# vice87/gam-ngs

Hardware: AMD Instinct MI355X
Metric: GCUPS (higher is better)
Workload: dtype int32 (fast blocks: exact packed-f16 offsets from per-lane int32 bases, two tasks per register; results bit-identical to the reference's int64 DP)

## Files before the change

### gam_ngs_amd/csrc/gamdp_dev.h

```cpp
#pragma once
#include <stdint.h>

namespace gamdp {

typedef uint32_t u32;
typedef uint64_t u64;

constexpr int SEQ_PAD_BASES = 4096;

#ifndef GAMDP_WAVES_PER_SIMD
#define GAMDP_WAVES_PER_SIMD 5
#endif

struct DevTask {
    const u32* a2;
    const u32* an;
    const u32* b2;
    const u32* bn;
    int64_t a_base;
    int64_t b_base;
    int64_t end_a;
    int32_t alen, blen;
    int32_t begin_a, begin_b;
    int32_t X;
    int32_t band;
    u32 flags;
    u32 res_idx;
    u64 ops_off;
    u64 ops_cap;
};

enum : u32 { TF_FORCE_START = 1, TF_FORCE_END = 2, TF_WANT_OPS = 4,
             TF_DIAG_SKIP_TRACEBACK = 8 ,
             TF_NO_DIRFREE = 16 ,
             TF_DIAG_COUNT_MAT = 32 ,
             TF_PADDING = 64 ,
             TF_CALL_N = 128  };

#ifdef GAMDP_DIAG
constexpr u32 TF_LIVE_MASK = ~0u;
#else
constexpr u32 TF_LIVE_MASK = ~(u32)(TF_DIAG_SKIP_TRACEBACK | TF_NO_DIRFREE | TF_DIAG_COUNT_MAT);
#endif

struct DevResult {
    int32_t begin_a, begin_b;
    int32_t score;
    u32 n_match, length;
    int32_t first_a, first_b, last_a, last_b;
    u32 flags;
};

struct LaunchParams {
    const DevTask* tasks;
    u32 n_tasks;
    u32* cursor;
    DevResult* results;
    uint8_t* ops_buf;
    u32* scratch;
    u64 slot_words;
    u64 dir_words;
    u32 ypad;
    u64 ckpt_off;
    u64 bnd_off;
    u32 flags;
    u32 prio_R, prio_from;
    u32* stats;
};
enum : int { LS_UNITS = 0, LS_DIRFREE, LS_PACKED_TOP, LS_PACKED_TOP_MIXED, LS_STRIPS, LS_TOP_WANTED, LS_SKIP_TESTS, LS_SKIP_TESTED, LS_SKIP_GROUPS, LS_SKIP_SHORT, LS_COUNT = 12 };
constexpr u32 LP_WALK_SKIP_DIAG = 32;
constexpr u32 LP_WALK_SIDE_BY_SIDE = 1;
constexpr u32 LP_NO_PACKED_TOP = 2;
constexpr u32 LP_NO_PACKED_TOP_MIXED = 16;
constexpr u32 LP_WALK_PRIO_SHIFT = 8;

enum KernelId : int {
    K_C17_CE4 = 0,
    K_C17_CE4_N,
    K_C5_CE0,
    K_C5_CE0_N,
    K_P17_CE4,
    K_O19_CE15,
    K_Q19_CE15,
    K_Q19_CE15_N,
    K_GEN_C2, K_GEN_C3, K_GEN_C5, K_GEN_C9, K_GEN_C17,
    K_WIDE,
    K_COUNT
};

constexpr int FAMILY_COLS[5] = {2, 3, 5, 9, 17};
constexpr int band_cols(const u32 band)
{
    for (int k = 0; k < 4; k++) if (2 * (u64)band + 1 <= 64u * (u64)FAMILY_COLS[k]) return FAMILY_COLS[k];
    return 17;
}
constexpr int cols_index(const int cols)
{
    for (int k = 0; k < 4; k++) if (FAMILY_COLS[k] == cols) return k;
    return 4;
}
static_assert(K_GEN_C3 == K_GEN_C2 + 1 && K_GEN_C5 == K_GEN_C2 + 2 && K_GEN_C9 == K_GEN_C2 + 3 && K_GEN_C17 == K_GEN_C2 + 4,
              "K_GEN_C2 .. K_GEN_C17: contiguous, in the order of FAMILY_COLS");
constexpr int gen_kernel_id(const int cols) { return (int)K_GEN_C2 + cols_index(cols); }

#if defined(__HIPCC__)
#define GAMDP_HD __host__ __device__
#else
#define GAMDP_HD
#endif

constexpr u32 PAT_OFF = 0x2000u, PAT_MIN = 0x0400u, PAT_MAX = 0x7BFFu - 21u;
GAMDP_HD inline u32 pat_encode(int rel) { return (PAT_OFF + (u32)rel) & 0xFFFFu; }
GAMDP_HD inline int pat_decode(u32 p16) { return (int)(int16_t)(uint16_t)p16 - (int)PAT_OFF; }

GAMDP_HD inline int preflight_hd(u64 alen, u64 blen, u64 band, u64 begin_a, u64 end_a, u64 begin_b, u64 end_b, bool fs, bool fe,
                                 u64* X_out, u64* cells_out)
{
    constexpr int64_t MAXGAP = 10;
    enum { S_OK = 0, S_EMPTY = 1, S_OOR = 2, S_INVALID = 3 };
    auto mn = [](int64_t x, int64_t y) { return x < y ? x : y; };
    *X_out = 0;
    *cells_out = 0;
    if (end_b < begin_b) return S_EMPTY;
    if (begin_a >= (1ull << 31) - 65536) return S_INVALID;
    const int64_t lo = ((int64_t)begin_a - (int64_t)band) > 0 ? ((int64_t)begin_a - (int64_t)band) : 0, hi = (int64_t)begin_a + (int64_t)band;
    if (begin_b >= blen) {
        bool any;
        if (!fs) any = lo < (int64_t)alen;
        else any = (lo <= mn(hi, MAXGAP)) || lo < (int64_t)alen;
        return any ? S_OOR : S_INVALID;
    }
    if (end_b >= blen) end_b = blen - 1;
    u64 X = end_b - begin_b + 1;
    const u64 lim = alen + band - begin_a;
    if (lim < X) X = lim;
    if (X > 500000) X = 500000;
    if (X == 0) return S_INVALID;
    const u64 Y = 2 * band + 1;
    *X_out = X;
    *cells_out = X * Y;
    if (fs) {
        const int64_t up = mn(hi, MAXGAP);
        if (lo <= up && up >= (int64_t)alen) return S_OOR;
    }
    if (begin_a > alen + band) {
        bool found = false;
        if (!fe) found = begin_a + (X - 1) - band <= end_a;
        {
            const bool ge = end_a >= begin_a + band;
            const int64_t i0 = ge ? (int64_t)(end_a - (begin_a + band)) : 0;
            const int64_t j0 = ge ? (int64_t)(2 * band) : (int64_t)(2 * band) - (int64_t)(begin_a + band - end_a);
            if (j0 >= 0 && (u64)i0 < X) {
                const int64_t kmax = mn((int64_t)X - 1 - i0, j0);
                if (!fe) found = true;
                else if (X >= (u64)MAXGAP + 1 && (u64)(i0 + kmax) >= X - 1 - (u64)MAXGAP) found = true;
            }
        }
        return found ? S_OOR : S_EMPTY;
    }
    return S_OK;
}

GAMDP_HD inline bool npre_window_has_n(const u32* pre, int64_t len, bool rc, u64 off, int64_t lo, int64_t hi)
{
    if (pre == nullptr) return false;
    const int64_t o_lo = (int64_t)off + (lo > 0 ? lo : 0), o_hi = ((int64_t)off + hi < len - 1) ? (int64_t)off + hi : len - 1;
    if (o_lo > o_hi) return false;
    const int64_t f_lo = rc ? len - 1 - o_hi : o_lo, f_hi = rc ? len - 1 - o_lo : o_hi;
    return pre[(f_hi / 256) + 1] != pre[f_lo / 256];
}
GAMDP_HD inline bool call_touches_n(const u32* pre_a, int64_t alen, bool a_rc, u64 a_off, const u32* pre_b, int64_t blen, bool b_rc, u64 b_off,
                                    int64_t band, int64_t begin_a, int64_t begin_b, int64_t X, int64_t margin)
{
    return npre_window_has_n(pre_a, alen, a_rc, a_off, begin_a - band - margin, begin_a + X - 1 + band + margin) ||
           npre_window_has_n(pre_b, blen, b_rc, b_off, begin_b - margin, begin_b + X - 1 + margin);
}

struct DevBlk { int32_t m_begin, m_end, s_begin, s_end; };
struct DevMB {
    const u32 *a2, *an;
    const u32 *b2, *bn;
    const u32 *b2rc, *bnrc;
    u64 mlen, slen;
    u64 m_start, s_start, s_end;
    u64 align_thr;
    u32 first_blk, n_blocks;
    u32 audit_first;
    u32 rows;
    u32 try_rev;
    u32 has_n;
    const u32 *npre_a, *npre_b;
    u32 max_x;
    u64 slot_off[2];
    u64 slot_words, dir_words;
    u64 ckpt_off, bnd_off;
};
struct ChainOut { u32 n_dp; u32 state; u32 t_begin, t_end; u32 hw, hw_twin; u32 t_end_att[2]; u32 t_begin2; u32 pad; };
struct ChainWin { u64 begin_a, end_a, begin_b, end_b; u32 X; u32 info; };
struct ChainSync { u32 verdict[2]; u32 n[2]; u32 fin; u32 cancel; u32 t_begin; u32 hw[2]; u32 t_end[2]; u32 t_begin2; };
struct ChainParams {
    const DevMB* mbs; const DevBlk* blks; u32 n_mbs;
    u32 n_twins;
    ChainSync* sync;
    u32 first_mb;
    u32* cursor;
    DevResult* audit; ChainOut* out;
    ChainWin* win;
    u32* scratch; u32 ypad; u32 band;
    u32 max_rows;
    DevResult* host_audit; ChainOut* host_out; u32* host_done; u32 epoch;
    ChainWin* host_win;
    u32 skew_call;
    int32_t n_margin;
    u32 n_by_contig;
};
int chain_slots_per_workgroup();

struct KernelInfo {
    KernelId id;
    const char* name;
    int cols;
    u32 band;
    int tasks_per_wave;
    int waves_per_cu;
    bool n_aware;
    bool dirfree;
    bool two_dir_images;
    int dir_block_words;
    int ckpt_words;
    int bnd_words;
    void (*kernel)(LaunchParams);
};
extern const KernelInfo kernel_info[K_COUNT];

inline u64 dir_words_for(const KernelInfo& ki, const u64 X, const u64 band)
{
    const u64 Y = 2 * band + 1;
    if (ki.id == K_WIDE) return X * Y;
    const u64 C = (u64)ki.cols, LE = (Y - 1) / C;
    const u64 extra = ki.tasks_per_wave > 1 ? 3 : 0;
    return ((X - 1 + LE) / 16 + 1 + extra) * (u64)ki.dir_block_words;
}
struct SlotGeom { u64 dir_words; u32 ypad; u64 slot_words, ckpt_off, bnd_off; };
inline SlotGeom slot_geom(const KernelInfo& ki, const u64 max_dir_words, const u32 max_band)
{
    SlotGeom g;
    g.ypad = ((2 * max_band + 2 + 63) / 64) * 64;
    g.dir_words = ((max_dir_words + 63) / 64) * 64;
    const u64 tpw = (u64)ki.tasks_per_wave;
    u64 ckpt_words = 0, bnd_words = 0;
    if (tpw > 1 || ki.dirfree) {
        const u64 nblk = g.dir_words / (u64)ki.dir_block_words + 1;
        ckpt_words = (nblk / 4 + 2) * (u64)ki.ckpt_words;
        bnd_words = (nblk + 4) * (u64)ki.bnd_words;
    }
    const u64 sides_end = (ki.two_dir_images ? 2 * g.dir_words : g.dir_words) + 4ull * g.ypad * tpw;
    g.slot_words = sides_end + ckpt_words + bnd_words;
    g.ckpt_off = ckpt_words ? sides_end : 0;
    g.bnd_off = g.ckpt_off + ckpt_words;
    return g;
}

struct KernelFamily {
    const void* kernel[5];
    const char* name[5];
    unsigned threads;
};
const KernelFamily& score_family();
const KernelFamily& carry_family();
const KernelFamily& chain_carry_family();
const KernelFamily& chain_gen_family();

enum ChainNBit : int {
    CHAIN_N_UNREPORTED,
    CHAIN_N_BY_WINDOW,
    CHAIN_N_EVERY_DP
};
struct ChainKernel {
    const char* name;
    const void* kernel;
    int cols;
    unsigned threads;
    const KernelInfo* slots;
    bool twins;
    ChainNBit n_bit;
};
const ChainKernel& chain2_kernel(bool has_n);
inline ChainKernel family_chain_kernel(const KernelFamily& f, const int cols, const KernelInfo* slots, const bool twins, const ChainNBit n_bit)
{
    return ChainKernel{f.name[cols_index(cols)], f.kernel[cols_index(cols)], cols, f.threads, slots, twins, n_bit};
}

int launch_align(int kid, const LaunchParams& p, unsigned n_slots, unsigned dyn_lds, void* stream);
int launch_wide(const LaunchParams& p, unsigned n_slots, void* stream);
constexpr int WIDE_WORKGROUPS_PER_CU = 8;

struct alignas(16) ScoreRec {
    int32_t score, end_a, end_b;
    u32 info;
};
struct ScoreParams {
    const DevTask* tasks;
    u32 n_tasks;
    u32* cursor;
    ScoreRec* results;
};

struct CarryParams {
    const DevTask* tasks;
    u32 n_tasks;
    u32* cursor;
    DevResult* results;
};
constexpr u32 CARRY_COLS_SHIFT = 16;


}
```

### gam_ngs_amd/csrc/kernel_pair.inc

```
#ifndef GAMDP_PACKED_TOP
#define GAMDP_PACKED_TOP 1
#endif
typedef _Float16 h2 __attribute__((ext_vector_type(2)));
__device__ __forceinline__ h2 as_h2(u32 x) { return __builtin_bit_cast(h2, x); }
__device__ __forceinline__ u32 as_u(h2 x) { return __builtin_bit_cast(u32, x); }
constexpr u32 PK_NINF = 0xFC00FC00u;
constexpr u32 PK_PINF = 0x7C007C00u;

__device__ __forceinline__ u32 pk(const _Float16 lo, const _Float16 hi) { const h2 v = {lo, hi}; return as_u(v); }
__device__ __forceinline__ _Float16 lo_of(const u32 v) { return as_h2(v).x; }
__device__ __forceinline__ _Float16 hi_of(const u32 v) { return as_h2(v).y; }

__device__ __forceinline__ _Float16 g4_to_h(const int g4, const int base)
{
    if (g4 <= NEG / 2) return lo_of(PK_NINF);
    return (_Float16)(float)((g4 >> 2) - base);
}
__device__ __forceinline__ int h_to_g4(const _Float16 h, const int base)
{
    const float f = (float)h;
    if (!(f > -60000.0f)) return NEG;
    if (!(f < 60000.0f)) return 0;
    return 4 * ((int)f + base);
}

typedef unsigned short us2 __attribute__((ext_vector_type(2)));
constexpr u32 PAT_OFF2 = PAT_OFF * 0x00010001u;
__device__ __forceinline__ u32 pat_add(const u32 a, const u32 b) { return __builtin_bit_cast(u32, __builtin_bit_cast(us2, a) + __builtin_bit_cast(us2, b)); }
__device__ __forceinline__ u32 pat_sub(const u32 a, const u32 b) { return __builtin_bit_cast(u32, __builtin_bit_cast(us2, a) - __builtin_bit_cast(us2, b)); }
__device__ __forceinline__ u32 pk16(const int lo, const int hi) { return ((u32)lo & 0xFFFFu) | ((u32)hi << 16); }
__device__ __forceinline__ u32 pat_lo(const u32 v) { return v & 0xFFFFu; }
__device__ __forceinline__ u32 pat_hi(const u32 v) { return v >> 16; }
__device__ __forceinline__ u32 g4_to_pat(const int g4, const int base)
{
    if (g4 <= NEG / 2) return 0xFC00u;
    return pat_encode((g4 >> 2) - base);
}
__device__ __forceinline__ int pat_to_g4(const u32 p, const int base)
{
    if (p & 0x8000u) return NEG;
    return 4 * (pat_decode(p) + base);
}
__device__ __forceinline__ u32 h2_to_pat(const u32 v)
{
    const h2 lim = {(_Float16)16000.0f, (_Float16)16000.0f};
    const h2 c = __builtin_elementwise_min(__builtin_elementwise_max(as_h2(v), -lim), lim);
    return pat_add(pk16((int)(short)c.x, (int)(short)c.y), PAT_OFF2);
}

template <int C, int LPT>
struct PairFmt {
    typedef Strip<LPT, true> ST;
    static constexpr bool GRP = (LPT == QL);
    static constexpr u32 CK_LANE = GRP ? 24u : (u32)LANE_WORDS<C>;
    static_assert(!GRP || C + 4 <= 24, "checkpoint row of the eight-task kernel");
    static constexpr u32 CK_ROWS = 64u * CK_LANE;
    static constexpr u32 CK_WORDS = GRP ? CK_ROWS : CK_ROWS + 128;
    static constexpr u32 BND_VALS = ST::BND_WORDS;
    static constexpr u32 BND_WORDS = GRP ? ST::BND_WORDS : ST::BND_WORDS + 2u * ST::NB;
    static constexpr int RC = 4;
};
__shared__ u32 s_ringB2[RING_B + ROWS];
__shared__ u32 s_pcap[QT][2][20];

__device__ __forceinline__ u32 pk_sel(const u32 codeA, const u32 codeB) { return 0x000C000Cu | (codeA << 8) | ((4u + codeB) << 24); }
__device__ __forceinline__ u32 pk_tab(const u32 codeb) { return 0x44444444u + (0x03u << (codeb * 8u)); }
__device__ __forceinline__ u32 pat_sel(const u32 codeA, const u32 codeB) { return 0x0C000C00u | codeA | ((4u + codeB) << 16); }
__device__ __forceinline__ u32 pat_tab(const u32 codeb) { return 0x0C0C0C0Cu + (0x09u << (codeb * 8u)); }

__device__ __forceinline__ u32 code2_at(gcptr p2, int64_t idx) { return (p2[idx >> 4] >> ((idx & 15) * 2)) & 3u; }

__shared__ u32 s_oB2[QT][64 + ROWS];
template <int C, int LPT, bool PAT = false>
struct PRing {
    static_assert(!PAT || LPT == 64, "the pattern format is the two-task kernel's");
    static __device__ __forceinline__ u32 sel(const u32 codeA, const u32 codeB) { return PAT ? pat_sel(codeA, codeB) : pk_sel(codeA, codeB); }
    static __device__ __forceinline__ u32 tab(const u32 codeb) { return PAT ? pat_tab(codeb) : pk_tab(codeb); }
    typedef typename std::conditional<LPT == 64, const u32*, const uint16_t*>::type APtr;
    static constexpr int SZ = QRing<C>::SZ;
    static __device__ __forceinline__ void put_a(const int sub, const int k, const u32 codeA, const u32 codeB)
    {
        if constexpr (LPT == 64) RingA<C>::put(k, sel(codeA, codeB));
        else {
            const u32 pos = (u32)k % (u32)SZ;
            const uint16_t v = (uint16_t)(codeA | ((4u + codeB) << 8));
            s_oA16[sub][pos] = v;
            if (pos < ROWS) s_oA16[sub][pos + SZ] = v;
        }
    }
    static __device__ __forceinline__ void put_b(const int sub, const int k, const u32 ta, const u32 tb)
    {
        if constexpr (LPT == 64) {
            const int pb = k & (RING_B - 1);
            s_ringB[pb] = ta; s_ringB2[pb] = tb;
            if (pb < ROWS) { s_ringB[pb + RING_B] = ta; s_ringB2[pb + RING_B] = tb; }
        } else {
            const int pb = k & 63;
            s_qB[sub][pb] = ta; s_oB2[sub][pb] = tb;
            if (pb < ROWS) { s_qB[sub][pb + 64] = ta; s_oB2[sub][pb + 64] = tb; }
        }
    }
    static __device__ __forceinline__ APtr a_lane(const int tau0, const int lane)
    {
        if constexpr (LPT == 64) return s_ringA + (u32)((tau0 + (C - 1) * (lane + 1)) >> 4) % (u32)RingA<C>::COLS;
        else return s_oA16[lane >> 4] + (u32)(tau0 + (C - 1) * ((lane & (QL - 1)) + 1)) % (u32)SZ;
    }
    static __device__ __forceinline__ u32 a_read(APtr p, const int r)
    {
        if constexpr (LPT == 64) return p[r * RingA<C>::COLS];
        else return __builtin_amdgcn_perm(0x0C0C0C0Cu, (u32)p[r], 0x01040004u);
    }
    static __device__ __forceinline__ const u32* b_lane(const int tau0, const int lane, const int half)
    {
        if constexpr (LPT == 64) return (half ? s_ringB2 : s_ringB) + ((tau0 - lane) & (RING_B - 1));
        else return (half ? s_oB2[lane >> 4] : s_qB[lane >> 4]) + ((tau0 - (lane & (QL - 1))) & 63);
    }
    template <int C2>
    static __device__ __forceinline__ _Float16 cap_pick(const int wlane, const int half, const u32 (&Lp)[C2], const int idx)
    {
        const int lane = wlane & (LPT - 1);
        if constexpr (LPT == 64) {
            u32* const cb = (u32*)s_cap[half][lane & 1];
#pragma unroll
            for (int c = 0; c < C2; ++c) cb[c] = Lp[c];
            const u32 v = cb[idx];
            return half ? hi_of(v) : lo_of(v);
        } else {
            u32* const cb = s_pcap[wlane >> 4][lane & 1];
#pragma unroll
            for (int c = 0; c < C2; ++c) cb[c] = Lp[c];
            return __builtin_bit_cast(_Float16, reinterpret_cast<const uint16_t*>(cb)[2 * idx + half]);
        }
    }
    template <int C2>
    static __device__ __forceinline__ u32 cap_pick_pat(const int wlane, const int half, const u32 (&Lp)[C2], const int idx)
    {
        static_assert(LPT == 64, "the pattern format is the two-task kernel's");
        u32* const cb = (u32*)s_cap[half][wlane & 1];
#pragma unroll
        for (int c = 0; c < C2; ++c) cb[c] = Lp[c];
        const u32 v = cb[idx];
        return half ? pat_hi(v) : pat_lo(v);
    }
    static constexpr u32 MARK_A = 13u, MARK_B = 9u;
    template <bool MARK = false>
    static __device__ __forceinline__ void produce(const int T, const int lane, const u32 awA, const u32 awB, const u32 bwA, const u32 bwB, const int km1A = 0, const int km1B = 0)
    {
        const int r = lane & (QL - 1);
        if (LPT == QL || lane < ROWS) {
            const int k = T + (C - 1) * LPT + r;
            u32 cA = (awA >> (2 * r)) & 3u, cB = (awB >> (2 * r)) & 3u;
            if constexpr (MARK) { cA = (k == km1A) ? MARK_A : cA; cB = (k == km1B) ? MARK_B : cB; }
            put_a(lane >> 4, k, cA, cB);
            put_b(lane >> 4, T + r, tab((bwA >> (2 * r)) & 3u), tab((bwB >> (2 * r)) & 3u));
        }
    }
    template <bool MARK = false>
    static __device__ __forceinline__ void prime(const Tk& ta, const Tk& tb, const int blk, const int lane, const int km1A = 0, const int km1B = 0)
    {
        const int T0 = blk * ROWS, tl = lane & (LPT - 1), sub = lane >> 4;
        const int64_t A0a = ta.a_base + ta.begin_a - ta.band, A0b = tb.a_base + tb.begin_a - tb.band;
        for (int k = T0 + tl; k < T0 + ROWS + (C - 1) * LPT; k += LPT) {
            u32 cA = code2_at(ta.a2, A0a + k), cB = code2_at(tb.a2, A0b + k);
            if constexpr (MARK) { cA = (k == km1A) ? MARK_A : cA; cB = (k == km1B) ? MARK_B : cB; }
            put_a(sub, k, cA, cB);
        }
        const int64_t Ba = ta.b_base + ta.begin_b, Bb = tb.b_base + tb.begin_b;
        for (int k = T0 - (LPT - 1) + tl; k <= T0 + ROWS - 1; k += LPT) put_b(sub, k, tab(code2_at(ta.b2, Ba + k)), tab(code2_at(tb.b2, Bb + k)));
    }
};

template <int C, bool HASN, bool UNTAGGED, int LPT>
__device__ __forceinline__ void single_prime(const Tk& t, const int blk, const int wlane, u32 (&W)[C + 15])
{
    typedef Ring<C, LPT, HASN> RG;
    const int T0 = blk * ROWS, lane = wlane & (LPT - 1), sub = wlane >> 4;
    const int64_t A0 = t.a_base + t.begin_a - t.band, BB = t.b_base + t.begin_b;
    for (int k = T0 + lane; k < T0 + ROWS + (C - 1) * LPT; k += LPT) RG::put_a(sub, k, code2_at(t.a2, A0 + k), false);
    for (int k = T0 - (LPT - 1) + lane; k <= T0 + ROWS - 1; k += LPT)
        RG::put_b(sub, k, enc_b<HASN>(code2_at(t.b2, BB + k), false) - (UNTAGGED ? RING_TAG<HASN> : 0u));
    const int64_t s0 = A0 + (int64_t)(C - 1) * lane + T0;
    const u32 ab = fetch16(t.a2, s0), ab2 = (C - 1 > 16) ? fetch16(t.a2, s0 + 16) : 0u;
#pragma unroll
    for (int k = 0; k < C - 1; ++k) W[k] = (k < 16) ? enc_a<HASN>((ab >> (2 * k)) & 3u, false) : enc_a<HASN>((ab2 >> (2 * (k - 16))) & 3u, false);
#pragma unroll
    for (int k = C - 1; k < C + 15; ++k) W[k] = 0;
}

template <int C, int LPT>
__device__ __forceinline__ void ck_store(gptr ck, const int wlane, const u32 (&Lp)[C], const int baseA, const int baseB)
{
    typedef PairFmt<C, LPT> FMT;
    if constexpr (FMT::GRP) {
        const u32 rA = (u32)lane_shl1<LPT>(baseA, baseA), rB = (u32)lane_shl1<LPT>(baseB, baseB);
        gptr row = ck + (u32)wlane * FMT::CK_LANE;
#pragma unroll
        for (int g = 0; g < 6; ++g) {
            auto w = [&](const int i) -> u32 { return i < C ? Lp[i < C ? i : 0] : (i == C ? (u32)baseA : (i == C + 1 ? (u32)baseB : (i == C + 2 ? rA : (i == C + 3 ? rB : 0u)))); };
            const u32x4 q = {w(4 * g), w(4 * g + 1), w(4 * g + 2), w(4 * g + 3)};
            *(g4ptr)(row + 4 * g) = q;
        }
    } else {
        img_store<C, true>(ck, wlane, Lp);
        ck[FMT::CK_ROWS + wlane] = (u32)baseA;
        ck[FMT::CK_ROWS + 64 + wlane] = (u32)baseB;
    }
}

template <int C, int LPT>
__device__ __forceinline__ int cap_limit(const Tk& t, const int lane) { return max(0, min(C, t.Y - C * lane)); }
template <int LPT>
__device__ __forceinline__ void cap_table(const int wlane, const int half, const int E0, const int R0, const int P0, const int L0)
{
    if ((wlane & (LPT - 1)) == 0) {
        const int4 e = {E0, R0, P0, L0};
        *reinterpret_cast<int4*>(s_captab[LPT == 64 ? 0 : wlane >> 4][half]) = e;
    }
}
template <int C, int CE, int LPT, bool LAST, bool PAT = false>
__device__ __forceinline__ void side_capture(const int wlane, const int half, const int T, const int base, const u32 (&Lp)[C], const int cap_max, giptr const cap_slot)
{
    const int lane = wlane & (LPT - 1);
    const int4 e = *reinterpret_cast<const int4*>(s_captab[LPT == 64 ? 0 : wlane >> 4][half]);
    const int cE = e.x - (C - 1) * lane - T;
    if ((u32)cE < (u32)cap_max && T <= e.y + lane) {
        if constexpr (PAT) {
            const u32 vE = PRing<C, LPT>::cap_pick_pat(wlane, half, Lp, cE);
            cap_slot[e.z - lane + T] = pat_decode(vE) + base + 8 * (lane - e.x - T);
        } else {
            const _Float16 vE = PRing<C, LPT>::cap_pick(wlane, half, Lp, cE);
            cap_slot[e.z - lane + T] = (int)(float)vE + base + 8 * (lane - e.x - T);
        }
    }
    if constexpr (LAST) {
        if (T == e.y + lane && cap_max > 0) {
            giptr const lp = cap_slot + (e.w + C * lane);
            const int k1 = base - 16 * e.y - 8 * C * lane;
            auto put = [&](const int c) __attribute__((always_inline)) {
                if constexpr (PAT) lp[c] = pat_decode(half ? pat_hi(Lp[c]) : pat_lo(Lp[c])) + (k1 - 8 * c);
                else lp[c] = (int)(float)(half ? hi_of(Lp[c]) : lo_of(Lp[c])) + (k1 - 8 * c);
            };
#pragma unroll
            for (int c = 0; c <= CE; ++c) put(c);
            if (cap_max == C) {
#pragma unroll
                for (int c = CE + 1; c < C; ++c) put(c);
            }
        }
    }
}

template <int C, int CE, bool END, int LPT = 64>
__device__ __noinline__ void pair_range(BlockState<C>* sta, BlockState<C>* stb, const Tk* tpa, const Tk* tpb, const int blk_begin_, const int blk_end_, const int wlane)
{
    static_assert(CE >= 0 && CE < C - 1 && (LPT == QL || (C - 1) % 16 == 0), "band 512 on 64 lanes (transposed ring A) or band 150 on 16");
    constexpr bool PAT = (LPT == 64);
    typedef PRing<C, LPT, PAT> PR;
    const Tk ta = load_tk<LPT>(tpa), tb = load_tk<LPT>(tpb);
    const int blk_begin = uni(blk_begin_), blk_end = uni(blk_end_);
    const int lane = wlane & (LPT - 1);
    const int LE = (ta.Y - 1) / C;
    u32 Lp[C], W[C + 15];
    int baseA, baseB;
    u32 Lin, dL, dR;
    {
        baseA = (sta->Lp[0] <= NEG / 2) ? 0 : (sta->Lp[0] >> 2);
        baseB = (stb->Lp[0] <= NEG / 2) ? 0 : (stb->Lp[0] >> 2);
        const int lA = __shfl_up(baseA, 1, LPT), lB = __shfl_up(baseB, 1, LPT), rA = __shfl_down(baseA, 1, LPT), rB = __shfl_down(baseB, 1, LPT);
        const bool hasL = lane >= 1 && lane <= LE, hasR = lane < LE;
        if constexpr (PAT) {
#pragma unroll
            for (int c = 0; c < C; ++c) Lp[c] = g4_to_pat(sta->Lp[c], baseA) | (g4_to_pat(stb->Lp[c], baseB) << 16);
            Lin = g4_to_pat(sta->Lin, baseA) | (g4_to_pat(stb->Lin, baseB) << 16);
            dL = hasL ? pk16(lA - baseA, lB - baseB) : 0u;
            dR = hasR ? pk16(rA - baseA, rB - baseB) : 0u;
        } else {
#pragma unroll
            for (int c = 0; c < C; ++c) Lp[c] = pk(g4_to_h(sta->Lp[c], baseA), g4_to_h(stb->Lp[c], baseB));
            Lin = pk(g4_to_h(sta->Lin, baseA), g4_to_h(stb->Lin, baseB));
            dL = hasL ? pk((_Float16)(float)(lA - baseA), (_Float16)(float)(lB - baseB)) : 0u;
            dR = hasR ? pk((_Float16)(float)(rA - baseA), (_Float16)(float)(rB - baseB)) : 0u;
        }
        const int T0 = blk_begin * ROWS;
        const int64_t sa = ta.a_base + ta.begin_a - ta.band + (int64_t)(C - 1) * lane + T0, sb = tb.a_base + tb.begin_a - tb.band + (int64_t)(C - 1) * lane + T0;
        const u32 wa = fetch16(ta.a2, sa), wb = fetch16(tb.a2, sb);
        const u32 wa2 = (C - 1 > 16) ? fetch16(ta.a2, sa + 16) : 0u, wb2 = (C - 1 > 16) ? fetch16(tb.a2, sb + 16) : 0u;
#pragma unroll
        for (int k = 0; k < C - 1; ++k)
            W[k] = (k < 16) ? PR::sel((wa >> (2 * k)) & 3u, (wb >> (2 * k)) & 3u) : PR::sel((wa2 >> (2 * (k - 16))) & 3u, (wb2 >> (2 * (k - 16))) & 3u);
#pragma unroll
        for (int k = C - 1; k < C + 15; ++k) W[k] = 0;
    }
    PR::prime(ta, tb, blk_begin, wlane);

    const int64_t iAa = ta.a_base + ta.begin_a - ta.band + (C - 1) * LPT, iBa = ta.b_base + ta.begin_b;
    const int64_t iAb = tb.a_base + tb.begin_a - tb.band + (C - 1) * LPT, iBb = tb.b_base + tb.begin_b;
    gcptr paA = ta.a2 + (iAa >> 4), pbA = ta.b2 + (iBa >> 4), paB = tb.a2 + (iAb >> 4), pbB = tb.b2 + (iBb >> 4);
    const u32 shaA = (u32)(iAa & 15) * 2u, shbA = (u32)(iBa & 15) * 2u, shaB = (u32)(iAb & 15) * 2u, shbB = (u32)(iBb & 15) * 2u;
    u32 aA_lo = paA[blk_begin + 1], aA_hi = paA[blk_begin + 2], bA_lo = pbA[blk_begin + 1], bA_hi = pbA[blk_begin + 2];
    u32 aB_lo = paB[blk_begin + 1], aB_hi = paB[blk_begin + 2], bB_lo = pbB[blk_begin + 1], bB_hi = pbB[blk_begin + 2];
    asm volatile("" : "+v"(aA_lo), "+v"(aA_hi), "+v"(bA_lo), "+v"(bA_hi), "+v"(aB_lo), "+v"(aB_hi), "+v"(bB_lo), "+v"(bB_hi));
    [[maybe_unused]] const h2 three = {(_Float16)3.0f, (_Float16)3.0f};
    const bool no_up = lane == LE;
    typedef Strip<LPT, true> ST;
    typedef PairFmt<C, LPT> FMT;
    constexpr int SPAN = (C - 1) * 21 + FMT::RC * ROWS * 21;
    static_assert(!PAT || ((int)PAT_OFF - (SPAN + 21) >= (int)PAT_MIN && (int)PAT_OFF + SPAN + 21 <= (int)PAT_MAX), "the live patterns of a group stay normal, finite f16 numbers");
    constexpr int NB = ST::NB, FI = ST::FI;
    const int sshift = uni(ta.sshift);
    const bool edge = ST::opens_strip(wlane, sshift);
    const u32 my_slot = ST::slot_of(wlane, sshift);
    const u64 edge_mask = __ballot(edge);
    u32* const s_bnd = ST::staging();
    u32* const sb = s_bnd + my_slot;
    gptr const ckpt = ta.ckpt, bnd = ta.bnd;
    int xkeep = (int)PK_NINF;
    const int prio_R = uni(ta.prio_R), prio_nblk = uni(ta.prio_nblk);
    const int cap_max = END ? cap_limit<C, LPT>(ta, lane) : 0;
    giptr const cap_slot = (giptr)unip(ta.dir);
    if constexpr (END) {
        cap_table<LPT>(wlane, 0, ta.eaRel, ta.X - 1, (int)(ta.adh - cap_slot) - ta.iA, (int)(ta.lastrow - cap_slot));
        cap_table<LPT>(wlane, 1, tb.eaRel, tb.X - 1, (int)(tb.adh - cap_slot) - tb.iA, (int)(tb.lastrow - cap_slot));
    }
    constexpr bool ROT = (C + 15 == 32);
    auto block_body = [&](auto phase, const int blk) __attribute__((always_inline)) {
        constexpr int WO = ROT ? 16 * decltype(phase)::value : 0;
#define WX(i) (ROT ? (((i) + WO) & 31) : (i))
        const int T = (blk + 1) * ROWS, tau0 = blk * ROWS;
        if (prio_R != 0 && (blk & 7) == 0) set_prio_by_remaining(prio_nblk - blk, prio_R);
        const u32 aA_nx = paA[blk + 3], bA_nx = pbA[blk + 3], aB_nx = paB[blk + 3], bB_nx = pbB[blk + 3];
        PR::produce(T, wlane, __builtin_amdgcn_alignbit(aA_hi, aA_lo, shaA), __builtin_amdgcn_alignbit(aB_hi, aB_lo, shaB),
                    __builtin_amdgcn_alignbit(bA_hi, bA_lo, shbA), __builtin_amdgcn_alignbit(bB_hi, bB_lo, shbB));
        if ((blk & 3) == 0) ck_store<C, LPT>(ckpt + (u64)(blk >> 2) * FMT::CK_WORDS, wlane, Lp, baseA, baseB);
        if constexpr (!FMT::GRP) {
            if (edge) {
                gptr bb = bnd + (u64)blk * FMT::BND_WORDS + FMT::BND_VALS;
                bb[my_slot] = (u32)baseA;
                bb[NB + my_slot] = (u32)baseB;
            }
        }
        const typename PR::APtr ringA_lane = PR::a_lane(tau0, wlane);
        const u32* const rbA = PR::b_lane(tau0, wlane, 0);
        const u32* const rbB = PR::b_lane(tau0, wlane, 1);
        {
            u32 tA[2], tB[2];
            u32 m[3], D[2];
            u32 L = Lin, x = PK_NINF, Lrecv = Lin;
            W[WX(C - 1)] = PR::a_read(ringA_lane, 0);
            tA[0] = rbA[0]; tB[0] = rbB[0];
            W[WX(C)] = PR::a_read(ringA_lane, 1);
            tA[1] = rbA[1]; tB[1] = rbB[1];
            auto do_perm = [&](const int g) __attribute__((always_inline)) {
                const int r = g / C, c = g % C;
                m[g % 3] = __builtin_amdgcn_perm(tB[r & 1], tA[r & 1], W[WX(r + c)]);
            };
            auto do_fma = [&](const int g) __attribute__((always_inline)) {
                if constexpr (PAT) D[g % 2] = m[g % 3] + Lp[g % C];
                else D[g % 2] = as_u(__builtin_elementwise_fma(as_h2(m[g % 3]), three, as_h2(Lp[g % C])));
            };
            auto do_max = [&](const int g) __attribute__((always_inline)) {
                const int c = g % C;
                h2 U = as_h2((c < C - 1) ? Lp[(c < C - 1) ? c + 1 : c] : x);
                if (c == CE) U = as_h2(no_up ? PK_NINF : as_u(U));
                L = as_u(__builtin_elementwise_maximum(__builtin_elementwise_maximum(as_h2(D[g % 2]), U), as_h2(L)));
                Lp[c] = L;
            };
            do_perm(0); do_perm(1); do_fma(0);
            __builtin_amdgcn_sched_barrier(0);
            static_for<ROWS>([&](auto rc) __attribute__((always_inline)) {
                constexpr int r = decltype(rc)::value;
#pragma unroll
                for (int c = 0; c < C; ++c) {
                    const int g = r * C + c;
                    if (c == 0) {
                        L = Lin; Lrecv = Lin;
                        do_fma(g + 1);
                        do_max(g);
                        do_perm(g + 2);
                    } else {
                        do_max(g);
                        if (g + 1 < ROWS * C) do_fma(g + 1);
                        if (g + 2 < ROWS * C) do_perm(g + 2);
                    }
                    if (c == 2) xkeep = lane_shl1<LPT>(xkeep, (int)Lp[0]);
                    if (c == 3) {
                        x = PAT ? pat_add((u32)xkeep, dR) : as_u(as_h2((u32)xkeep) + as_h2(dR));
                        lds_store2_masked<4 * (r % FI) * NB, 4 * (NB * FI + (r % FI) * NB)>(sb, Lrecv, Lp[0], edge_mask);
                    }
                    __builtin_amdgcn_sched_barrier(0);
                }
                if constexpr (r + 2 < ROWS) { W[WX(C + 1 + r)] = PR::a_read(ringA_lane, r + 2); tA[r & 1] = rbA[r + 2]; tB[r & 1] = rbB[r + 2]; }
                Lin = (u32)lane_shr1<LPT>((int)Lin, (int)L);
                Lin = PAT ? pat_add(Lin, dL) : as_u(as_h2(Lin) + as_h2(dL));
                __builtin_amdgcn_sched_barrier(0);
                if constexpr (END) {
                    side_capture<C, CE, LPT, true, PAT>(wlane, 0, tau0 + r, baseA, Lp, cap_max, cap_slot);
                    side_capture<C, CE, LPT, true, PAT>(wlane, 1, tau0 + r, baseB, Lp, cap_max, cap_slot);
                }
                if ((r % FI) == FI - 1) {
                    constexpr u32 PER = 2u * NB * FI / 64u;
                    const u32 w0 = (u32)wlane * PER;
                    const u32* src = s_bnd + ST::staging_index(w0);
                    gptr bp = bnd + (u64)blk * FMT::BND_WORDS + (u32)(r / FI) * (u32)(2 * NB * FI) + w0;
#pragma unroll
                    for (u32 k = 0; k < PER; k += 4) {
                        const u32x4 v = {src[k * NB], src[(k + 1) * NB], src[(k + 2) * NB], src[(k + 3) * NB]};
                        *(g4ptr)(bp + k) = v;
                    }
                }
            });
        }
#ifdef GAMDP_DIAG
        {
            if constexpr (PAT) {
                auto mn = [](const u32 a, const u32 b) { return __builtin_bit_cast(u32, __builtin_elementwise_min(__builtin_bit_cast(us2, a), __builtin_bit_cast(us2, b))); };
                auto mx = [](const u32 a, const u32 b) { return __builtin_bit_cast(u32, __builtin_elementwise_max(__builtin_bit_cast(us2, a), __builtin_bit_cast(us2, b))); };
                u32 nIn = 0xFFFFFFFFu, xIn = 0, nOut = 0xFFFFFFFFu, xOut = 0;
#pragma unroll
                for (int c = 0; c < C; ++c) {
                    if (c <= CE) { nIn = mn(nIn, Lp[c]); xIn = mx(xIn, Lp[c]); }
                    else { nOut = mn(nOut, Lp[c]); xOut = mx(xOut, Lp[c]); }
                }
                if (lane >= 1) { nIn = mn(nIn, Lin); xIn = mx(xIn, Lin); }
                const u32 xv = pat_add((u32)xkeep, dR);
                if (blk > blk_begin) { nOut = mn(nOut, xv); xOut = mx(xOut, xv); }
                if (lane < LE) { nIn = mn(nIn, nOut); xIn = mx(xIn, xOut); }
                if (lane <= LE) {
                    if (pat_lo(nIn) < PAT_MIN || pat_lo(xIn) > PAT_MAX) ta.pos0[-1] = 1;
                    if (pat_hi(nIn) < PAT_MIN || pat_hi(xIn) > PAT_MAX) tb.pos0[-1] = 1;
                }
            } else {
            u32 mIn = 0, mOut = 0;
#pragma unroll
            for (int c = 0; c < C; ++c) {
                const u32 a = Lp[c] & 0x7FFF7FFFu;
                if (c <= CE) mIn = as_u(__builtin_elementwise_max(as_h2(mIn), as_h2(a)));
                else mOut = as_u(__builtin_elementwise_max(as_h2(mOut), as_h2(a)));
            }
            if (lane >= 1) mIn = as_u(__builtin_elementwise_max(as_h2(mIn), as_h2(Lin & 0x7FFF7FFFu)));
            const u32 xv = as_u(as_h2((u32)xkeep) + as_h2(dR)) & 0x7FFF7FFFu;
            if (blk > blk_begin) mOut = as_u(__builtin_elementwise_max(as_h2(mOut), as_h2(xv)));
            if (lane < LE) mIn = as_u(__builtin_elementwise_max(as_h2(mIn), as_h2(mOut)));
            if (lane <= LE) {
                if (!((float)lo_of(mIn) < 2040.0f)) ta.pos0[-1] = 1;
                if (!((float)hi_of(mIn) < 2040.0f)) tb.pos0[-1] = 1;
            }
            }
        }
#endif
        if constexpr (PAT) {
            if ((blk & (FMT::RC - 1)) == FMT::RC - 1 || blk + 1 == blk_end) {
                const u32 d = (lane <= LE) ? pat_sub(Lp[0], PAT_OFF2) : 0u;
                baseA += (int)(short)pat_lo(d);
                baseB += (int)d >> 16;
#pragma unroll
                for (int c = 0; c < C; ++c) Lp[c] = pat_sub(Lp[c], d);
                if (lane != 0) Lin = pat_sub(Lin, d);
                const u32 dl = (u32)lane_shr1<LPT>((int)d, (int)d);
                const u32 dr = (u32)lane_shl1<LPT>((int)d, (int)d);
                if (lane >= 1 && lane <= LE) dL = pat_sub(pat_add(dL, dl), d);
                if (lane < LE) dR = pat_sub(pat_add(dR, dr), d);
            }
        } else
        if ((blk & (FMT::RC - 1)) == FMT::RC - 1 || blk + 1 == blk_end) {
            const float fa = (float)lo_of(Lp[0]), fb = (float)hi_of(Lp[0]);
            const bool oka = fa > -60000.0f && fa < 60000.0f, okb = fb > -60000.0f && fb < 60000.0f;
            const u32 d = pk(oka ? lo_of(Lp[0]) : (_Float16)0.0f, okb ? hi_of(Lp[0]) : (_Float16)0.0f);
            baseA += oka ? (int)fa : 0;
            baseB += okb ? (int)fb : 0;
#pragma unroll
            for (int c = 0; c < C; ++c) Lp[c] = as_u(as_h2(Lp[c]) - as_h2(d));
            Lin = as_u(as_h2(Lin) - as_h2(d));
            const u32 dl = (u32)lane_shr1<LPT>((int)d, (int)d);
            const u32 dr = (u32)lane_shl1<LPT>((int)d, (int)d);
            if (lane >= 1 && lane <= LE) dL = as_u(as_h2(dL) + as_h2(dl) - as_h2(d));
            if (lane < LE) dR = as_u(as_h2(dR) + as_h2(dr) - as_h2(d));
        }
        if constexpr (!ROT) {
#pragma unroll
            for (int k = 0; k < C - 1; ++k) W[k] = W[k + ROWS];
        }
        aA_lo = aA_hi; aA_hi = aA_nx; bA_lo = bA_hi; bA_hi = bA_nx;
        aB_lo = aB_hi; aB_hi = aB_nx; bB_lo = bB_hi; bB_hi = bB_nx;
#undef WX
    };
    if constexpr (ROT) {
        int blk = blk_begin;
        for (; blk + 1 < blk_end; blk += 2) {
            block_body(std::integral_constant<int, 0>{}, blk);
            block_body(std::integral_constant<int, 1>{}, blk + 1);
        }
        if (blk < blk_end) block_body(std::integral_constant<int, 0>{}, blk);
    } else {
        for (int blk = blk_begin; blk < blk_end; ++blk) block_body(std::integral_constant<int, 0>{}, blk);
    }
    const bool dead_lane = PAT && lane > LE;
    auto back = [&](const u32 v, const int half, const int base) -> int {
        if constexpr (PAT) return dead_lane ? NEG : pat_to_g4(half ? pat_hi(v) : pat_lo(v), base);
        else return h_to_g4(half ? hi_of(v) : lo_of(v), base);
    };
#pragma unroll
    for (int c = 0; c < C; ++c) {
        sta->Lp[c] = back(Lp[c], 0, baseA); stb->Lp[c] = back(Lp[c], 1, baseB);
        sta->acc[c] = 0; stb->acc[c] = 0;
    }
    sta->Lin = back(Lin, 0, baseA); stb->Lin = back(Lin, 1, baseB);
    sta->Lout = sta->Lp[C - 1]; stb->Lout = stb->Lp[C - 1];
}

template <int C, int CE, int LPT = 64, bool FS = false>
__device__ __noinline__ void pair_top_range(BlockState<C>* sta, BlockState<C>* stb, const Tk* tpa, const Tk* tpb, const int blk_begin_, const int blk_end_, const int wlane)
{
    static_assert(CE >= 0 && CE < C - 1 && (LPT == QL || (C - 1) % 16 == 0), "band 512 on 64 lanes (transposed ring A) or band 150 on 16");
    typedef PRing<C, LPT> PR;
    const Tk ta = load_tk<LPT>(tpa), tb = load_tk<LPT>(tpb);
    const int blk_begin = uni(blk_begin_), blk_end = uni(blk_end_);
    const int lane = wlane & (LPT - 1);
    const int LE = (ta.Y - 1) / C;
    const int T0 = blk_begin * ROWS;
    const int km1A = ta.band - ta.begin_a - 1, km1B = tb.band - tb.begin_a - 1;
    const int zk = 8 * km1A, zkB = 8 * km1B;
    u32 Lp[C], W[C + 15];
    int baseA, baseB;
    u32 Lin, dL, dR;
    {
        const int rp = T0 - lane - 1, p0 = ta.begin_a + rp + C * lane - ta.band;
        const int p0B = tb.begin_a + rp + C * lane - tb.band;
        const bool dead0 = p0 < -1 && lane <= LE;
        const bool dead0B = p0B < -1 && lane <= LE;
        baseA = (sta->Lp[0] <= NEG / 2) ? 0 : (sta->Lp[0] >> 2);
        baseB = (stb->Lp[0] <= NEG / 2) ? 0 : (stb->Lp[0] >> 2);
        if (dead0) baseA = 16 * rp + 8 * C * lane;
        if (dead0B) baseB = 16 * rp + 8 * C * lane;
#pragma unroll
        for (int c = 0; c < C; ++c) {
            const bool dead = p0 + c < -1 && lane <= LE, deadB = p0B + c < -1 && lane <= LE;
            Lp[c] = pk(dead ? lo_of(PK_NINF) : g4_to_h(sta->Lp[c], baseA), deadB ? lo_of(PK_NINF) : g4_to_h(stb->Lp[c], baseB));
        }
        Lin = pk(dead0 ? lo_of(PK_NINF) : g4_to_h(sta->Lin, baseA), dead0B ? lo_of(PK_NINF) : g4_to_h(stb->Lin, baseB));
        const int lA = __shfl_up(baseA, 1, LPT), lB = __shfl_up(baseB, 1, LPT), rA = __shfl_down(baseA, 1, LPT), rB = __shfl_down(baseB, 1, LPT);
        const bool hasL = lane >= 1 && lane <= LE, hasR = lane < LE;
        dL = hasL ? pk((_Float16)(float)(lA - baseA), (_Float16)(float)(lB - baseB)) : 0u;
        dR = hasR ? pk((_Float16)(float)(rA - baseA), (_Float16)(float)(rB - baseB)) : 0u;
        const int64_t sa = ta.a_base + ta.begin_a - ta.band + (int64_t)(C - 1) * lane + T0, sb = tb.a_base + tb.begin_a - tb.band + (int64_t)(C - 1) * lane + T0;
        const u32 wa = fetch16(ta.a2, sa), wb = fetch16(tb.a2, sb);
        const u32 wa2 = (C - 1 > 16) ? fetch16(ta.a2, sa + 16) : 0u, wb2 = (C - 1 > 16) ? fetch16(tb.a2, sb + 16) : 0u;
        const int w0k = (C - 1) * lane + T0;
#pragma unroll
        for (int k = 0; k < C - 1; ++k) {
            const u32 cA = (k < 16) ? (wa >> (2 * k)) & 3u : (wa2 >> (2 * (k - 16))) & 3u, cB = (k < 16) ? (wb >> (2 * k)) & 3u : (wb2 >> (2 * (k - 16))) & 3u;
            W[k] = pk_sel((w0k + k == km1A) ? PR::MARK_A : cA, (w0k + k == km1B) ? PR::MARK_B : cB);
        }
#pragma unroll
        for (int k = C - 1; k < C + 15; ++k) W[k] = 0;
    }
    PR::template prime<true>(ta, tb, blk_begin, wlane, km1A, km1B);
    const int64_t iAa = ta.a_base + ta.begin_a - ta.band + (C - 1) * LPT, iBa = ta.b_base + ta.begin_b;
    const int64_t iAb = tb.a_base + tb.begin_a - tb.band + (C - 1) * LPT, iBb = tb.b_base + tb.begin_b;
    gcptr paA = ta.a2 + (iAa >> 4), pbA = ta.b2 + (iBa >> 4), paB = tb.a2 + (iAb >> 4), pbB = tb.b2 + (iBb >> 4);
    const u32 shaA = (u32)(iAa & 15) * 2u, shbA = (u32)(iBa & 15) * 2u, shaB = (u32)(iAb & 15) * 2u, shbB = (u32)(iBb & 15) * 2u;
    u32 aA_lo = paA[blk_begin + 1], aA_hi = paA[blk_begin + 2], bA_lo = pbA[blk_begin + 1], bA_hi = pbA[blk_begin + 2];
    u32 aB_lo = paB[blk_begin + 1], aB_hi = paB[blk_begin + 2], bB_lo = pbB[blk_begin + 1], bB_hi = pbB[blk_begin + 2];
    const h2 three = {(_Float16)3.0f, (_Float16)3.0f};
    const bool no_up = lane == LE;
    typedef Strip<LPT, true> ST;
    typedef PairFmt<C, LPT> FMT;
    constexpr int NB = ST::NB, FI = ST::FI;
    const int sshift = uni(ta.sshift);
    const bool edge = ST::opens_strip(wlane, sshift);
    const u32 my_slot = ST::slot_of(wlane, sshift);
    const u64 edge_mask = __ballot(edge);
    u32* const s_bnd = ST::staging();
    u32* const sb = s_bnd + my_slot;
    gptr const ckpt = ta.ckpt, bnd = ta.bnd;
    int xkeep = (int)PK_NINF;
    auto hf = [](const int v) -> _Float16 { return (_Float16)(float)v; };
    int g0A = baseA, g0B = baseB;
    const int cap_max = cap_limit<C, LPT>(ta, lane);
    giptr const cap_slot = (giptr)unip(ta.dir);
    cap_table<LPT>(wlane, 0, ta.band - ta.begin_a, ta.X - 1, (int)(ta.pos0 - cap_slot), 0);
    cap_table<LPT>(wlane, 1, tb.band - tb.begin_a, tb.X - 1, (int)(tb.pos0 - cap_slot), 0);
    for (int blk = blk_begin; blk < blk_end; ++blk) {
        const int T = (blk + 1) * ROWS, tau0 = blk * ROWS;
        const u32 aA_nx = paA[blk + 3], bA_nx = pbA[blk + 3], aB_nx = paB[blk + 3], bB_nx = pbB[blk + 3];
        PR::template produce<true>(T, wlane, __builtin_amdgcn_alignbit(aA_hi, aA_lo, shaA), __builtin_amdgcn_alignbit(aB_hi, aB_lo, shaB),
                                   __builtin_amdgcn_alignbit(bA_hi, bA_lo, shbA), __builtin_amdgcn_alignbit(bB_hi, bB_lo, shbB), km1A, km1B);
        if ((blk & 3) == 0) {
            if constexpr (LPT == 64) {
                u32 Pp[C];
#pragma unroll
                for (int c = 0; c < C; ++c) Pp[c] = h2_to_pat(Lp[c]);
                ck_store<C, LPT>(ckpt + (u64)(blk >> 2) * FMT::CK_WORDS, wlane, Pp, baseA, baseB);
            } else ck_store<C, LPT>(ckpt + (u64)(blk >> 2) * FMT::CK_WORDS, wlane, Lp, baseA, baseB);
            g0A = baseA; g0B = baseB;
        }
        if constexpr (!FMT::GRP) {
            if (edge) {
                gptr bb = bnd + (u64)blk * FMT::BND_WORDS + FMT::BND_VALS;
                bb[my_slot] = (u32)baseA;
                bb[NB + my_slot] = (u32)baseB;
            }
        }
        const u32 Kpk = FMT::GRP ? pk(hf(baseA - g0A), hf(baseB - g0B)) : 0u;
        const typename PR::APtr ringA_lane = PR::a_lane(tau0, wlane);
        const u32* const rbA = PR::b_lane(tau0, wlane, 0);
        const u32* const rbB = PR::b_lane(tau0, wlane, 1);
        static_for<ROWS>([&](auto rc) __attribute__((always_inline)) {
            constexpr int r = decltype(rc)::value;
            W[C - 1 + r] = PR::a_read(ringA_lane, r);
            const u32 tabA = rbA[r], tabB = rbB[r];
            const int row = tau0 + r - lane;
            const int zg = 8 * row + zk, zgB = 8 * row + zkB;
            const bool zA = row <= km1A && lane <= LE, zB = row <= km1B && lane <= LE;
            const u32 Z = pk(zA ? hf(min(max(zg - baseA, -60000), 60000)) : lo_of(PK_NINF), zB ? hf(min(max(zgB - baseB, -60000), 60000)) : lo_of(PK_NINF));
            u32 ZL = Z;
            if constexpr (FS) {
                const bool gA = ta.fs && row > FORCE_MAXGAP, gB = tb.fs && row > FORCE_MAXGAP;
                ZL = (gA ? 0x0000FC00u : (Z & 0x0000FFFFu)) | (gB ? 0xFC000000u : (Z & 0xFFFF0000u));
            }
            const u32 Lrecv = Lin;
            u32 L = Lin, x = PK_NINF;
            auto cell = [&](const int c) __attribute__((always_inline)) {
                const u32 m = __builtin_amdgcn_perm(tabB, tabA, W[r + c]);
                const h2 D = __builtin_elementwise_fma(as_h2(m), three, as_h2(Lp[c]));
                h2 U = as_h2((c < C - 1) ? Lp[(c < C - 1) ? c + 1 : c] : x);
                if (c == CE) U = as_h2(no_up ? PK_NINF : as_u(U));
                L = as_u(__builtin_elementwise_maximum(__builtin_elementwise_maximum(D, U), as_h2(L)));
                Lp[c] = as_u(__builtin_elementwise_max(as_h2(L), as_h2(Z)));
                L = FS ? as_u(__builtin_elementwise_max(as_h2(L), as_h2(ZL))) : Lp[c];
            };
            cell(0);
            xkeep = lane_shl1<LPT>(xkeep, (int)Lp[0]);
            x = as_u(as_h2((u32)xkeep) + as_h2(dR));
            lds_store2_masked<4 * (r % FI) * NB, 4 * (NB * FI + (r % FI) * NB)>(sb, FMT::GRP ? as_u(as_h2(Lrecv) + as_h2(Kpk)) : h2_to_pat(Lrecv),
                                                                               FMT::GRP ? as_u(as_h2(Lp[0]) + as_h2(Kpk)) : h2_to_pat(Lp[0]), edge_mask);
#pragma unroll
            for (int c = 1; c < C; ++c) cell(c);
            Lin = (u32)lane_shr1<LPT>((int)Lin, (int)L);
            Lin = as_u(as_h2(Lin) + as_h2(dL));
            side_capture<C, CE, LPT, false>(wlane, 0, tau0 + r, baseA, Lp, cap_max, cap_slot);
            side_capture<C, CE, LPT, false>(wlane, 1, tau0 + r, baseB, Lp, cap_max, cap_slot);
            if ((r % FI) == FI - 1) {
                constexpr u32 PER = 2u * NB * FI / 64u;
                const u32 w0 = (u32)wlane * PER;
                const u32* src = s_bnd + ST::staging_index(w0);
                gptr bp = bnd + (u64)blk * FMT::BND_WORDS + (u32)(r / FI) * (u32)(2 * NB * FI) + w0;
#pragma unroll
                for (u32 k = 0; k < PER; k += 4) {
                    const u32x4 v = {src[k * NB], src[(k + 1) * NB], src[(k + 2) * NB], src[(k + 3) * NB]};
                    *(g4ptr)(bp + k) = v;
                }
            }
        });
        {
            const float fa = (float)lo_of(Lp[0]), fb = (float)hi_of(Lp[0]);
            const int rpn = T - lane - 1;
            const bool followA = lane <= LE && ta.begin_a + rpn + C * lane - ta.band < -1, followB = lane <= LE && tb.begin_a + rpn + C * lane - tb.band < -1;
            const bool oka = !followA && fa > -60000.0f && fa < 60000.0f, okb = !followB && fb > -60000.0f && fb < 60000.0f;
            const _Float16 step = (_Float16)(float)(16 * ROWS);
            const u32 d = pk(oka ? lo_of(Lp[0]) : (followA ? step : (_Float16)0.0f), okb ? hi_of(Lp[0]) : (followB ? step : (_Float16)0.0f));
            baseA += oka ? (int)fa : (followA ? 16 * ROWS : 0);
            baseB += okb ? (int)fb : (followB ? 16 * ROWS : 0);
#pragma unroll
            for (int c = 0; c < C; ++c) Lp[c] = as_u(as_h2(Lp[c]) - as_h2(d));
            Lin = as_u(as_h2(Lin) - as_h2(d));
            const u32 dl = (u32)lane_shr1<LPT>((int)d, (int)d);
            const u32 dr = (u32)lane_shl1<LPT>((int)d, (int)d);
            if (lane >= 1 && lane <= LE) dL = as_u(as_h2(dL) + as_h2(dl) - as_h2(d));
            if (lane < LE) dR = as_u(as_h2(dR) + as_h2(dr) - as_h2(d));
        }
#pragma unroll
        for (int k = 0; k < C - 1; ++k) W[k] = W[k + ROWS];
        aA_lo = aA_hi; aA_hi = aA_nx; bA_lo = bA_hi; bA_hi = bA_nx;
        aB_lo = aB_hi; aB_hi = aB_nx; bB_lo = bB_hi; bB_hi = bB_nx;
    }
#pragma unroll
    for (int c = 0; c < C; ++c) {
        sta->Lp[c] = h_to_g4(lo_of(Lp[c]), baseA); stb->Lp[c] = h_to_g4(hi_of(Lp[c]), baseB);
        sta->acc[c] = 0; stb->acc[c] = 0;
    }
    sta->Lin = h_to_g4(lo_of(Lin), baseA); stb->Lin = h_to_g4(hi_of(Lin), baseB);
    sta->Lout = sta->Lp[C - 1]; stb->Lout = stb->Lp[C - 1];
}

template <int C, bool HASN, bool UNTAGGED, int LPT = 64>
__device__ __noinline__ void single_resume(BlockState<C>* st, const Tk* tp, const int blk_, const int lane)
{
    const Tk t = load_tk<LPT>(tp);
    u32 W[C + 15];
    single_prime<C, HASN, UNTAGGED, LPT>(t, uni(blk_), lane, W);
#pragma unroll
    for (int k = 0; k < C - 1; ++k) st->W[k] = W[k];
}
```

Baseline: 15490.

## Use one wave-uniform base per task in the packed-pattern path, dropping neighbour deltas

In the 16-bit pattern path, the per-lane int32 bases become wave-uniform, taken from lane 0's values at load and at each renormalisation. The per-lane neighbour offsets dL/dR are then always zero, so the shuffles, pattern adds in the inner row loop, and the delta bookkeeping at renormalisation are removed. Because patterns must now span the whole band's range from one base, PAT_OFF is lowered and the static asserts are reworked to bound the wider span. The trade-off is less headroom before values leave the normal f16 range, which may trigger fallbacks more often.

```diff
diff --git a/gam_ngs_amd/csrc/gamdp_dev.h b/gam_ngs_amd/csrc/gamdp_dev.h
--- a/gam_ngs_amd/csrc/gamdp_dev.h
+++ b/gam_ngs_amd/csrc/gamdp_dev.h
@@ -109,7 +109,7 @@
 #define GAMDP_HD
 #endif
 
-constexpr u32 PAT_OFF = 0x2000u, PAT_MIN = 0x0400u, PAT_MAX = 0x7BFFu - 21u;
+constexpr u32 PAT_OFF = 0x1000u, PAT_MIN = 0x0400u, PAT_MAX = 0x7BFFu - 21u;
 GAMDP_HD inline u32 pat_encode(int rel) { return (PAT_OFF + (u32)rel) & 0xFFFFu; }
 GAMDP_HD inline int pat_decode(u32 p16) { return (int)(int16_t)(uint16_t)p16 - (int)PAT_OFF; }
 
diff --git a/gam_ngs_amd/csrc/kernel_pair.inc b/gam_ngs_amd/csrc/kernel_pair.inc
--- a/gam_ngs_amd/csrc/kernel_pair.inc
+++ b/gam_ngs_amd/csrc/kernel_pair.inc
@@ -262,19 +262,19 @@
     const int LE = (ta.Y - 1) / C;
     u32 Lp[C], W[C + 15];
     int baseA, baseB;
-    u32 Lin, dL, dR;
+    u32 Lin;
+    [[maybe_unused]] u32 dL = 0, dR = 0;
     {
         baseA = (sta->Lp[0] <= NEG / 2) ? 0 : (sta->Lp[0] >> 2);
         baseB = (stb->Lp[0] <= NEG / 2) ? 0 : (stb->Lp[0] >> 2);
-        const int lA = __shfl_up(baseA, 1, LPT), lB = __shfl_up(baseB, 1, LPT), rA = __shfl_down(baseA, 1, LPT), rB = __shfl_down(baseB, 1, LPT);
-        const bool hasL = lane >= 1 && lane <= LE, hasR = lane < LE;
         if constexpr (PAT) {
+            baseA = uni(baseA); baseB = uni(baseB);
 #pragma unroll
             for (int c = 0; c < C; ++c) Lp[c] = g4_to_pat(sta->Lp[c], baseA) | (g4_to_pat(stb->Lp[c], baseB) << 16);
             Lin = g4_to_pat(sta->Lin, baseA) | (g4_to_pat(stb->Lin, baseB) << 16);
-            dL = hasL ? pk16(lA - baseA, lB - baseB) : 0u;
-            dR = hasR ? pk16(rA - baseA, rB - baseB) : 0u;
         } else {
+            const int lA = __shfl_up(baseA, 1, LPT), lB = __shfl_up(baseB, 1, LPT), rA = __shfl_down(baseA, 1, LPT), rB = __shfl_down(baseB, 1, LPT);
+            const bool hasL = lane >= 1 && lane <= LE, hasR = lane < LE;
 #pragma unroll
             for (int c = 0; c < C; ++c) Lp[c] = pk(g4_to_h(sta->Lp[c], baseA), g4_to_h(stb->Lp[c], baseB));
             Lin = pk(g4_to_h(sta->Lin, baseA), g4_to_h(stb->Lin, baseB));
@@ -304,8 +304,11 @@
     const bool no_up = lane == LE;
     typedef Strip<LPT, true> ST;
     typedef PairFmt<C, LPT> FMT;
-    constexpr int SPAN = (C - 1) * 21 + FMT::RC * ROWS * 21;
-    static_assert(!PAT || ((int)PAT_OFF - (SPAN + 21) >= (int)PAT_MIN && (int)PAT_OFF + SPAN + 21 <= (int)PAT_MAX), "the live patterns of a group stay normal, finite f16 numbers");
+    constexpr int Y_MAX = C * LPT, SLACK = 64;
+    constexpr int SPAN_LO = (LPT - 1) * 21 + 21 + SLACK;
+    constexpr int SPAN_HI = (Y_MAX - 1) * 21 + (LPT - 1) * 21 + FMT::RC * ROWS * 21 + 21 + SLACK;
+    static_assert(!PAT || ((int)PAT_OFF - SPAN_LO >= (int)PAT_MIN + 1024 && (int)PAT_OFF + SPAN_HI + 1024 <= (int)PAT_MAX), "the live patterns of a task stay normal, finite f16 numbers, with a binade to spare");
+    static_assert(!PAT || -1024 - (int)PAT_OFF < -SPAN_LO, "\"no source\" decodes below every live value");
     constexpr int NB = ST::NB, FI = ST::FI;
     const int sshift = uni(ta.sshift);
     const bool edge = ST::opens_strip(wlane, sshift);
@@ -384,14 +387,14 @@
                     }
                     if (c == 2) xkeep = lane_shl1<LPT>(xkeep, (int)Lp[0]);
                     if (c == 3) {
-                        x = PAT ? pat_add((u32)xkeep, dR) : as_u(as_h2((u32)xkeep) + as_h2(dR));
+                        x = PAT ? (u32)xkeep : as_u(as_h2((u32)xkeep) + as_h2(dR));
                         lds_store2_masked<4 * (r % FI) * NB, 4 * (NB * FI + (r % FI) * NB)>(sb, Lrecv, Lp[0], edge_mask);
                     }
                     __builtin_amdgcn_sched_barrier(0);
                 }
                 if constexpr (r + 2 < ROWS) { W[WX(C + 1 + r)] = PR::a_read(ringA_lane, r + 2); tA[r & 1] = rbA[r + 2]; tB[r & 1] = rbB[r + 2]; }
                 Lin = (u32)lane_shr1<LPT>((int)Lin, (int)L);
-                Lin = PAT ? pat_add(Lin, dL) : as_u(as_h2(Lin) + as_h2(dL));
+                if constexpr (!PAT) Lin = as_u(as_h2(Lin) + as_h2(dL));
                 __builtin_amdgcn_sched_barrier(0);
                 if constexpr (END) {
                     side_capture<C, CE, LPT, true, PAT>(wlane, 0, tau0 + r, baseA, Lp, cap_max, cap_slot);
@@ -422,7 +425,7 @@
                     else { nOut = mn(nOut, Lp[c]); xOut = mx(xOut, Lp[c]); }
                 }
                 if (lane >= 1) { nIn = mn(nIn, Lin); xIn = mx(xIn, Lin); }
-                const u32 xv = pat_add((u32)xkeep, dR);
+                const u32 xv = (u32)xkeep;
                 if (blk > blk_begin) { nOut = mn(nOut, xv); xOut = mx(xOut, xv); }
                 if (lane < LE) { nIn = mn(nIn, nOut); xIn = mx(xIn, xOut); }
                 if (lane <= LE) {
@@ -450,16 +453,14 @@
 #endif
         if constexpr (PAT) {
             if ((blk & (FMT::RC - 1)) == FMT::RC - 1 || blk + 1 == blk_end) {
-                const u32 d = (lane <= LE) ? pat_sub(Lp[0], PAT_OFF2) : 0u;
-                baseA += (int)(short)pat_lo(d);
-                baseB += (int)d >> 16;
+                const u32 p0 = (u32)uni((int)Lp[0]);
+                const int dA = (int)(short)(pat_lo(p0) - PAT_OFF), dB = (int)(short)(pat_hi(p0) - PAT_OFF);
+                const u32 d = pk16(dA, dB);
+                baseA += dA;
+                baseB += dB;
 #pragma unroll
                 for (int c = 0; c < C; ++c) Lp[c] = pat_sub(Lp[c], d);
                 if (lane != 0) Lin = pat_sub(Lin, d);
-                const u32 dl = (u32)lane_shr1<LPT>((int)d, (int)d);
-                const u32 dr = (u32)lane_shl1<LPT>((int)d, (int)d);
-                if (lane >= 1 && lane <= LE) dL = pat_sub(pat_add(dL, dl), d);
-                if (lane < LE) dR = pat_sub(pat_add(dR, dr), d);
             }
         } else
         if ((blk & (FMT::RC - 1)) == FMT::RC - 1 || blk + 1 == blk_end) {
```

Result: no change. 15360 (-0.8%).
